# BirchKwok/lynsedb

Hardware: AMD Instinct MI355X
Metric: queries/sec, FLAT-IP 10000000x768 float32, batch=256, k=10 (higher is better)
Workload: dtype f32

## Files before the change

### lynsedb_amd/csrc/lynse_hip.hip

```cpp
#include <algorithm>
#include <atomic>
#include <chrono>
#include <cmath>
#include <cstdio>
#include <cstring>
#include <functional>
#include <condition_variable>
#include <memory>
#include <mutex>
#include <shared_mutex>
#include <string>
#include <thread>
#include <type_traits>
#include <vector>
#include <sched.h>

#include "kernels.h"
#include "scan_qs.h"
#include "scan_qh.h"
#include "ivf.h"
#include "pq.h"
#include "rabitq.h"
#include "range.h"
#include "additive.h"
// ... 913 lines not shown
    size_t seen = granted.load(std::memory_order_acquire);
    if (bytes <= seen) return LYNSE_OK;
    for (;;) {
        LY_TRY(set_max_lds(K, bytes));
        if (granted.compare_exchange_strong(seen, bytes, std::memory_order_acq_rel, std::memory_order_acquire)) return LYNSE_OK;
        bytes = std::max(bytes, seen);
    }
}
template <auto K, typename... Args>
static int launch_lds(dim3 grid, dim3 block, size_t lds, hipStream_t st, const Args&... a) {
    LY_TRY(ensure_lds<K>(lds));
    hipLaunchKernelGGL(K, grid, block, lds, st, a...);
    LY_HIP(hipGetLastError());
    return LYNSE_OK;
}

template <H16Cfg C>
static int launch_h16(dim3 grid, hipStream_t st, const ScanArgs& a) {
    return launch_lds<k_scan_h16<C.wq, C.wr, C.tq, C.tr, C.metric, C.nsv, C.nsq, C.nt_hint, C.tiled, C.rag, C.dbg, C.filt, C.i8q, C.emit, C.place, C.dense, C.prio, C.qcreg, C.fs>>(
        grid, h16_threads(C), h16_lds_bytes(C), st, a);
}
template <QsCfg C>
static int launch_qs(dim3 grid, hipStream_t st, const ScanArgs& a) {
    return launch_lds<k_scan_qs<C.nslab, C.rb, C.sl, C.ns, C.xpf, C.nbuf, C.dbg, C.ping, C.sts, C.met, C.smp, C.msk, C.f4>>(grid, QS_THREADS, qs_lds_bytes(C), st, a);
}
template <QhCfg C>
static int launch_qh(dim3 grid, hipStream_t st, const ScanArgs& a) {
    return launch_lds<k_scan_qh<C.nslab, C.met, C.ns, C.nbuf, C.qb, C.smp>>(grid, QH_THREADS, qh_lds_bytes(C), st, a);
}
template <class C, class T, class V, class... More>
constexpr C with(C c, T C::*member, V value, More... more) {
    c.*member = value;
    if constexpr (sizeof...(more) > 0) return with(c, more...);
    else return c;
}
template <class F>
static int with_metric(int metric, F&& f) {
    switch (metric) {
    case M_IP: return f(std::integral_constant<int, M_IP>{});
    case M_L2: return f(std::integral_constant<int, M_L2>{});
    default: return f(std::integral_constant<int, M_COS>{});
    }
}
template <H16Cfg BASE, int... VALUES>
static int dispatch_dbg(int dbg, dim3 grid, hipStream_t st, const ScanArgs& a) {
    int rc = LYNSE_OK;
    const bool known = (... || (dbg == VALUES ? (rc = launch_h16<with(BASE, &H16Cfg::dbg, VALUES)>(grid, st, a), true) : false));
// ... 327 lines not shown
    if (only768 || qs_variant() != 1) return false;
    if (!qs_widths_on()) return false;
    return ((nslab >= 2 && nslab <= 5) || nslab == 8) && ld == nslab * 128u;
}
static bool sts_env_on() { return env_on("LYNSE_HIP_STS", false); }
static bool qs_scan_ok(const ScanArgs& a, bool fs, bool filt, bool f4) {
    const int v = qs_variant();
    if (v < 1 || v > 3) return false;
    if (filt && (!qs_masked_on() || v == 2 || !a.mask || a.row_ids)) return false;
    if (f4) {
        return env_on("LYNSE_HIP_QS_F4", true) && v == 1 && !fs && !filt && a.emit_all == 0 && (a.nslab == 2 || a.nslab == 4 || a.nslab == 8) && a.ld16 == a.nslab * 128u &&
               a.qpad == 256 && a.nq <= 256 &&
               a.tile_stride == 0 && !a.mask && !a.row_ids && a.row1 > a.row0;
    }
    return !fs && a.emit_all == 0 && qs_width_ok(a.ld16, a.nslab, filt) && a.qpad == 256 && a.nq <= 256 && a.tile_stride == 0 &&
           (filt || (a.skip_stride == 0 && !a.mask)) && !a.row_ids && a.row1 > a.row0;
}
static uint32_t qs_grid(const ScanArgs& a, uint32_t num_cu) {
    const uint32_t rt = a.nslab == 8 ? 32u : qs_rows(qs_variant());
    const int e = env_int("LYNSE_HIP_SCAN_CUS", 0);
    const uint32_t cus = e > 0 ? std::min<uint32_t>((uint32_t)e, num_cu) : num_cu;
    return std::min<uint32_t>((a.row1 - a.row0 + rt - 1) / rt, cus);
}
static int launch_scan_qs(const ScanArgs& a, uint32_t grid, hipStream_t st) {
    if (a.dyn_thr)
        return launch_qs<with(QS_768, &QsCfg::ping, 0, &QsCfg::sts, 1)>(grid, st, a);
    if (a.mask) return launch_qs<with(QS_768, &QsCfg::msk, 1)>(grid, st, a);
    if (a.nslab >= 2 && a.nslab <= 5)
        return with_qs_slabs(a.nslab, [&](auto n) { return launch_qs<qs_64(decltype(n)::value)>(grid, st, a); });
    if (a.nslab == 8) return launch_qs<QS_1024>(grid, st, a);
    switch (qs_variant()) {
    case 2: return launch_qs<QsCfg{.nslab = 6, .rb = 1, .sl = 6, .ns = 6, .xpf = true, .nbuf = 8}>(grid, st, a);
    case 3: return launch_qs<with(QS_768, &QsCfg::ping, 0)>(grid, st, a);
    default: return launch_qs<QS_768>(grid, st, a);
    }
}

static bool qs_sample_ok(const ScanArgs& a, bool fs, bool filt, bool f4, uint32_t plan_tile) {
    const int v = qs_variant();
    if (!env_on("LYNSE_HIP_QS_SAMPLE", true) || (v != 1 && v != 3)) return false;
    return !fs && !filt && !f4 && a.emit_all == 2 && plan_tile == 256 && a.nslab != 8 && qs_width_ok(a.ld16, a.nslab) && a.qpad == 256 && a.nq <= 256 && a.tile_stride >= 256 &&
           a.skip_stride == 0 && !a.mask && !a.row_ids && a.row1 > a.row0;
}
static int launch_scan_qs_sample(const ScanArgs& a, uint32_t grid, hipStream_t st) {
    return with_qs_slabs(a.nslab, [&](auto n) { return launch_qs<with(qs_64(decltype(n)::value), &QsCfg::ping, 0, &QsCfg::smp, 1)>(grid, st, a); });
}

constexpr int QH_DEFAULT = 1;
static int qh_variant() { return env_int("LYNSE_HIP_QH", QH_DEFAULT); }
static bool qh_shape(uint32_t ld16, uint64_t nq) { return qh_variant() == 1 && nq > SCAN_BQ_SMALL && nq <= QCHUNK && (ld16 == 64u || ld16 == 128u); }
// ... 11 lines not shown
static int launch_scan_qh_any(const ScanArgs& a, int metric, uint32_t grid, hipStream_t st) {
    auto by_metric = [&](auto n) {
        return with_metric(metric, [&](auto m) { return launch_qh<qh_64(decltype(n)::value, decltype(m)::value, SMP)>(grid, st, a); });
    };
    return a.nslab == 1 ? by_metric(std::integral_constant<int, 1>{}) : by_metric(std::integral_constant<int, 2>{});
}
static int launch_scan_qh(const ScanArgs& a, int metric, uint32_t grid, hipStream_t st) { return launch_scan_qh_any<0>(a, metric, grid, st); }

static bool qh_sample_ok(const ScanArgs& a, bool filt, uint32_t qchunks, int level, uint32_t plan_tile) {
    if (!env_on("LYNSE_HIP_QH_SAMPLE", true) || qh_variant() != 1 || level != 0) return false;
    return !filt && a.emit_all == 2 && plan_tile == 256 && qchunks == 1 && a.qpad == 256 && a.nq <= 256 && a.tile_stride >= 256 && a.skip_stride == 0 && !a.mask && !a.row_ids &&
           !a.tiles && a.row1 > a.row0 && (a.nslab == 1 || a.nslab == 2) && a.ld16 == a.nslab * 64u;
}
static uint32_t qh_sample_grid(const ScanArgs& a, uint32_t sample_tiles, bool filt, uint32_t qchunks, int level, uint32_t plan_tile, uint32_t k, uint32_t cap, uint32_t num_cu) {
    if (!sample_tiles || !qh_sample_ok(a, filt, qchunks, level, plan_tile)) return 0;
    const uint32_t nt64 = sample_tiles * 4u, sgrid = std::min<uint32_t>(nt64, 2u * num_cu);
    const bool ok = (uint64_t)sgrid * 4u >= 8ull * k && sgrid * 4u <= cap && (nt64 + sgrid - 1) / sgrid <= 32u;
    return ok ? sgrid : 0u;
}
static int launch_scan_qh_sample(const ScanArgs& a, int metric, uint32_t grid, hipStream_t st) { return launch_scan_qh_any<1>(a, metric, grid, st); }

constexpr H16Cfg I8C_256 = with(F16_IP_256, &H16Cfg::rag, false, &H16Cfg::i8q, 2, &H16Cfg::emit, 0);
constexpr H16Cfg I8C_AG = with(I8C_256, &H16Cfg::wr, 2, &H16Cfg::tr, 4);
static int launch_scan_i8c(const ScanArgs& a, uint32_t grid, hipStream_t st, bool fs = false, bool filt = false, bool f4 = false, bool qs = false) {
    if (qs && f4) {
        if (a.nslab == 2) return launch_qs<with(qs_64(2), &QsCfg::f4, 1)>(grid, st, a);
        if (a.nslab == 8) return launch_qs<with(QS_1024, &QsCfg::f4, 1)>(grid, st, a);
        return launch_qs<with(qs_64(4), &QsCfg::f4, 1)>(grid, st, a);
    }
    if (qs) return launch_scan_qs(a, grid, st);
#ifdef LYNSE_EXPERIMENTS
    if (a.ld16 % 128 == 0 && a.emit_all == 0 && ((a.debug_flags >> 8) & 31)) {
        return dispatch_dbg<I8C_256, 3, 4, 8, 12, 7, 11, 1, 13, 14, 2, 16>((a.debug_flags >> 8) & 31, grid, st, a);
    }
#endif
    if (f4) {
        if (a.ld16 % 128 != 0 || filt || fs) return set_error(LYNSE_ERR_INTERNAL, "the FP4 Hamming scan runs unfiltered over whole slabs");
        if (a.emit_all == 1) return launch_h16<with(I8C_256, &H16Cfg::i8q, 3, &H16Cfg::emit, 1)>(grid, st, a);
        if (a.emit_all == 2) return launch_h16<with(I8C_256, &H16Cfg::i8q, 3, &H16Cfg::emit, 2)>(grid, st, a);
        if (a.dense) return launch_h16<with(I8C_256, &H16Cfg::i8q, 3, &H16Cfg::dense, true)>(grid, st, a);
        return launch_h16<with(I8C_256, &H16Cfg::i8q, 3)>(grid, st, a);
    }
    if (filt) {
        if (a.ld16 % 128 != 0 || a.row_ids) return set_error(LYNSE_ERR_INTERNAL, "the masked int8 scan needs whole 128-column slabs and a row bitmask");
        if (a.emit_all == 1) return launch_h16<with(I8C_256, &H16Cfg::filt, true, &H16Cfg::emit, 1)>(grid, st, a);
        if (a.emit_all != 0 || !a.dense) return set_error(LYNSE_ERR_INTERNAL, "the masked int8 scan runs emit-all and DENSE threshold stages");
        return launch_h16<with(I8C_256, &H16Cfg::filt, true, &H16Cfg::dense, true)>(grid, st, a);
    }
    if (ag_env() && a.ld16 % 128 == 0 && a.emit_all == 0 && !fs) {
        if (a.dense) return launch_h16<with(I8C_AG, &H16Cfg::dense, true)>(grid, st, a);
        return launch_h16<I8C_AG>(grid, st, a);
    }
    if (a.ld16 % 128 == 0) {
// ... 242 lines not shown
#else
    constexpr int w16env = -1;
#endif
    const bool filt = mask != nullptr || row_ids != nullptr;
    const int waves16 = l2n ? 0 : i8c ? 3 : (w16env >= 0 ? w16env : ((metric == M_IP && !filt) ? 3 : 0));
    const bool can_threshold_only = h16 && !binary && !filt && !no_lane_max_env() && k <= 128;
    Stage assign_stage{0u, (uint32_t)h->n};
    assign_stage.sample_tiles = (uint32_t)((h->n + 255) / 256);
    assign_stage.sample_stride = 256;
    const std::vector<Stage> plan = tl_assign ? std::vector<Stage>{assign_stage}
                                    : (sts || tl_coarse_dump) ? std::vector<Stage>{Stage{0u, (uint32_t)h->n}}
                                        : make_plan(h, k, (level == 0 && (!plan_tile || no_sample)) ? 1 : level, plan_tile, can_threshold_only,
                                                    (h16 && !i8c && !binary && k >= 64) ? 4u : 0u);
    const Stage sample = (!plan.empty() && plan[0].sample_tiles) ? plan[0] : Stage{0, 0};
    *sampled_plan = sample.sample_tiles != 0;
    const uint32_t sample_keys_per_tile = (small || mid64 || mid128 || waves16 != 0) ? 16u : 8u;
    const bool sample_threshold_only = h16 && !binary && !filt && sample.sample_tiles && !no_lane_max_env() && sample_keys_per_tile &&
                                       (k <= sample_keys_per_tile || (uint64_t)sample.sample_tiles * sample_keys_per_tile >= 8ull * k);
    const int fs_env = fused_sample_env();
    const bool fs = fs_env != 0 && !debug_flags_env() && i8c && !aug && !cosq && !l2n && !bin_mfma && !mid64 && !mid128 && h->ld8 % 128 == 0 && sample_threshold_only && plan.size() >= 2 && k <= 32 &&
                    sample.sample_tiles == (uint32_t)h->num_cu && (plan[1].r1 - plan[1].r0 + 255) / 256 >= (uint32_t)h->num_cu &&
                    (uint64_t)k * 50000ull > (uint64_t)sample.sample_tiles * plan_tile &&
                    dense_env_now() != 0;
    bool plan_used_segments = false, plan_used_qs = false, plan_qs_sample = false, plan_used_qh = false;
    const int fused_tail_env = env_int("LYNSE_HIP_FUSED_TAIL", 1);
    const bool fused_tail = fused_tail_env != 0 && !plan.empty();
    SelectArgs sa_last{};
    for (size_t si = 0; si < plan.size(); ++si) {
        const Stage s = plan[si];
        const bool emit_all = si == 0 && !sts;
        if (fs && si == 0) continue;
        const bool fs_stage = fs && si == 1;
        uint32_t qs_sample_keys = 0;
        hipEvent_t e0 = nullptr, e1 = nullptr;
        if (tl_prof) {
            LY_TRY(get_event(h, (*ev_used)++, &e0));
            LY_TRY(get_event(h, (*ev_used)++, &e1));
            LY_HIP(hipEventRecord(e0, st));
        }
        uint32_t st_nseg = 0, st_seg = 0;
        int a_emit_all_last = -1;
        if (binary && !bin_mfma) {
            BinArgs b{};
            b.P = h->packed; b.W = h->words; b.row0 = s.r0; b.row1 = s.r1; b.QW = w.QW; b.nq = nq;
            b.thr = w.thr; b.cand = w.cand; b.count = w.count; b.cap = w.cap; b.emit_all = emit_all ? 1 : 0;
            b.mask = mask;
            static const int rows_minq = env_int("LYNSE_HIP_BIN_ROWS_MINQ", 1);
// ... 84 lines not shown
                    a.dyn_warm = h->n >= 4000000ull ? 4u : 2u;
                }
                if (s.sample_tiles && !sts && qs_sample_ok(a, fs_stage, filt, bin_mfma, plan_tile)) {
                    const uint32_t nt64 = s.sample_tiles * 4u;
                    const uint32_t sgrid = std::min<uint32_t>(nt64, (uint32_t)h->num_cu);
                    if ((uint64_t)sgrid * 4u >= 8ull * k && sgrid * 4u <= w.cap && (nt64 + sgrid - 1) / sgrid <= 32u) {
                        a.ntiles = nt64;
                        LY_TRY(launch_scan_qs_sample(a, sgrid, st));
                        qs_sample_keys = sgrid * 4u;
                        plan_qs_sample = true;
                    }
                }
                if (!qs_sample_keys) {
                const bool qs = sts || (!ag && qs_scan_ok(a, fs_stage, filt, bin_mfma));
                uint32_t launch_grid = qs ? qs_grid(a, (uint32_t)h->num_cu) : grid;
                if (sts) {
                    const uint32_t nt = (a.row1 - a.row0 + 63) / 64;
                    uint32_t pitch = (nt + launch_grid - 1) / launch_grid;
                    auto gcd = [](uint32_t x, uint32_t y) { while (y) { const uint32_t t = x % y; x = y; y = t; } return x; };
                    while (gcd(pitch, k) != 1) ++pitch;
                    a.dyn_pitch = pitch;
                    launch_grid = (nt + pitch - 1) / pitch;
                }
                if (qs) { seg_geometry(launch_grid, 2, &a.nseg, &a.seg); plan_used_qs = true; }
                else
                if (!a.emit_all) seg_geometry(grid, (a.dense ? 8 : 4) / (ag ? 2 : 1), &a.nseg, &a.seg);
                if (fs_stage) {
                    a.fs_stride = sample.sample_stride; a.fs_rows = (uint32_t)h->n; a.gsync = w.gsync; a.Qf = Qf; a.marg2 = w.marg2;
                    a.thr_out = w.thr; a.k = k; a.ip_form = ip_form; a.metric = metric;
                    if (env_str("LYNSE_HIP_FS_STAMPS")) a.debug_flags |= 128;
                }
                LY_TRY(launch_scan_i8c(a, launch_grid, st, fs_stage, filt, bin_mfma, qs));
                }
            } else if (h16) {
                a.candB = w.candB; a.segcnt = w.segcnt;
                if (small) {
                    const uint32_t grid = std::min<uint32_t>(a.ntiles, (uint32_t)h->num_cu * 2);
                    if (!a.emit_all) seg_geometry(grid, 4, &a.nseg, &a.seg);
                    LY_TRY((launch_scan_h16<F16_SMALL>(a, metric, grid, st)));
                } else if (const uint32_t sgrid = qh_sample_grid(a, s.sample_tiles, filt, qchunks, level, plan_tile, k, w.cap, (uint32_t)h->num_cu)) {
                    a.ntiles = s.sample_tiles * 4u;
                    LY_TRY(launch_scan_qh_sample(a, metric, sgrid, st));
                    qs_sample_keys = sgrid * 4u;
                    plan_used_qh = true;
                } else if (qh_scan_ok(a, filt, qchunks, level)) {
                    uint32_t segs = 0;
                    const uint32_t grid = qh_grid(a, (uint32_t)h->num_cu, &segs);
                    seg_geometry(grid, segs, &a.nseg, &a.seg);
                    plan_used_qh = true;
                    LY_TRY(launch_scan_qh(a, metric, grid, st));
                } else {
                    const uint32_t grid = std::min<uint32_t>(a.ntiles, (uint32_t)h->num_cu);
                    const uint64_t seen_before = s.sample_tiles ? 0 : (sample.sample_tiles ? std::max<uint64_t>((uint64_t)sample.sample_tiles * plan_tile, s.r0) : s.r0);
                    a.dense = (!a.emit_all && waves16 == 0 && metric != M_IP && !filt && seen_before && (dense_env() >= 0 ? dense_env() != 0 : true)) ? 1 : 0;
                    if (!a.emit_all) seg_geometry(grid, a.dense ? 4 : ((waves16 == 3 || waves16 == 2) ? 4 : 2), &a.nseg, &a.seg);
// ... 64 lines not shown
        sa.emit_all_n = emit_all ? (s.sample_tiles ? (int)(s.sample_tiles * plan_tile) : (int)(s.r1 - s.r0)) : -1;
        if (!binary && emit_all && sample_threshold_only) {
            sa.threshold_only = 1;
            sa.drop_sentinels = 1;
            sa.emit_all_n = qs_sample_keys ? (int)qs_sample_keys : (int)(s.sample_tiles * sample_keys_per_tile);
        }
        sa.Qf = Qf; sa.V = score_rows(h); sa.ld = score_ld(h); sa.D = h->dim;
        sa.candB = w.candB; sa.segcnt = w.segcnt; sa.seg = st_seg; sa.nseg = st_nseg;
        sa.abort_word = fs_stage ? w.gsync + 2 : nullptr;
        if (sel_stamps_on())
            sa.stamps = reinterpret_cast<unsigned long long*>(w.gsync + 64) + (size_t)si * 256 * 8;
        if (fs_stage && env_str("LYNSE_HIP_DEBUG_FS")) return LYNSE_OK;
        if (fused_tail && si + 1 == plan.size()) { sa_last = sa; continue; }
        sa.lds_bytes = sel_lds_bytes(w.cap, nq);
        hipLaunchKernelGGL(k_select<SEL_NT>, dim3(nq), dim3(SEL_NT), sa.lds_bytes, st, sa);
        LY_HIP(hipGetLastError());
    }
    if (tl_prof && (!binary || bin_mfma)) {
        const uint64_t tiling = plan_used_qs ? 0x81u : plan_used_qh ? 0x82u : (small || mid64) ? 0x14u : ((mid128 || waves16 == 3 || waves16 == 2) ? 0x24u : 0x42u);
        std::lock_guard<std::mutex> plk(h->prof_mu);
        h->prof.last_plan = (sample.sample_tiles ? 1u : 0u) | ((sample.sample_tiles && sample_threshold_only) ? 2u : 0u) | (i8c ? 4u : 0u) |
                            (plan_used_segments ? 8u : 0u) | (small ? 16u : 0u) | (fs ? 128u : 0u) | ((uint64_t)(plan.size() & 0xff) << 8) | (tiling << 16) |
                            (sts ? (1ull << 24) : 0ull) | (plan_qs_sample ? (1ull << 25) : 0ull) |
                            (sq7 ? (1ull << 26) : 0ull);
    }
    FinalArgs fa{};
    fa.cand = w.cand; fa.count = w.count; fa.k = k; fa.out_k = out_k; fa.cap = w.cap; fa.metric = key_metric; fa.ip_form = ip_form;
    fa.ham_dim = bin_mfma ? h->dim : 0u;
    fa.neg_metric1 = (aug || cosq) ? metric + 1 : 0;
    fa.exact = binary ? 1 : 0; fa.Qf = Qf; fa.V = score_rows(h); fa.ld = score_ld(h); fa.D = h->dim;
    fa.row_stride = h->row_stride; fa.row_offset = h->row_offset;
    fa.nan_rows = (!binary && !mask && !row_ids && h->n <= 0xffffffffull) ? (uint32_t)h->n : 0u;
    fa.out_rows = r_dst ? r_dst : w.out_rows; fa.out_dists = d_dst ? d_dst : w.out_dists; fa.out_counts = w.out_counts;
    fa.out_counts2 = c2_dst;
    fa.pool_total = tl_prof ? w.pool_total : nullptr;
    fa.overflow = w.overflow; fa.any_overflow = any_ovf;
    if (hdr_direct) { fa.h_hdr = w.h_hdr; fa.hdr_q = w.qcap; }
    if (fused_tail) {
        TailArgs ta{sa_last, fa};
        ta.s.hand_exact = env_int("LYNSE_HIP_HAND_EXACT", 1);
        ta.s.lds_bytes = ta.f.lds_bytes = sel_lds_bytes(w.cap, nq);
        hipLaunchKernelGGL(k_select_final<SEL_NT>, dim3(nq), dim3(SEL_NT), ta.s.lds_bytes, st, ta);
        LY_HIP(hipGetLastError());
        (void)asc;
        return LYNSE_OK;
    }
    if (i8c && !bin_mfma) {
// ... 1406 lines not shown
```

### lynsedb_amd/csrc/scan_qs.h

```cpp
#pragma once

namespace lynse {

typedef int qs_i32x4 __attribute__((ext_vector_type(4)));
typedef int qs_i32x16 __attribute__((ext_vector_type(16)));

constexpr int QS_STS_LDS = 8 * 256 + 8 * 256;

struct QsCfg {
    int nslab, rb, sl, ns;
    bool xpf;
    int nbuf;
    int dbg = 0, ping = 0, sts = 0, met = 0, smp = 0, msk = 0, f4 = 0;
};
constexpr int QS_THREADS = 512;
constexpr size_t qs_lds_bytes(QsCfg c) {
    const size_t norm_slot = c.met == 1 ? (c.rb * 32 == 64 ? 256 : 1024) : 0;
    return (size_t)c.ns * c.sl * (c.rb * 32) * 128 + (c.sts ? QS_STS_LDS : 0) + (size_t)(c.ns + 1) * norm_slot;
}

template <int NSLAB, int RB, int SL, int NS, bool XPF, int NBUF, int DBG = 0, int PING = 0, int STS = 0, int MET = 0, int SMP = 0, int MSK = 0, int F4 = 0>
__global__ void __launch_bounds__(512, 2) k_scan_qs(ScanArgs a) {
    static_assert(NSLAB % SL == 0, "a tile is a whole number of steps");
    constexpr int TS = NSLAB / SL;
    constexpr int RT = RB * 32;
    constexpr int SB = SL * RT * 128;
    constexpr int PP = SB / 1024;
    static_assert(PP % 8 == 0, "the pieces of a stage split evenly over the 8 waves");
    constexpr int PPW = PP / 8;
    constexpr int NM = SL * 4 * RB;
    static_assert(NM % NBUF == 0 && NBUF >= 2 && NBUF <= NM, "fragment ring");
    static_assert(NS >= (XPF ? 4 : 3), "ring depth");
    constexpr int NRM = MET == 1 ? (RT == 64 ? 256 : 1024) : 0;
    constexpr int NRM_SLOTS = NS + 1;
    constexpr int NRM_OFF = NS * SB + (STS ? QS_STS_LDS : 0);
    static_assert(MET == 0 || (STS == 0 && TS == 1 && RT <= 256), "L2: whole-K stages; one dword / dwordx4 LDS-DMA brings a tile's norms");
    static_assert(NRM_OFF + NRM_SLOTS * NRM <= 160 * 1024, "LDS");
    static_assert((size_t)(NRM_OFF + NRM_SLOTS * NRM) <= qs_lds_bytes(QsCfg{NSLAB, RB, SL, NS, XPF, NBUF, DBG, PING, STS, MET, SMP, MSK, F4}),
                  "the LDS the body addresses ends inside what the launch asks for");
    static_assert(PING == 0 || TS == 1, "ping-pong: one step per tile");
    static_assert(STS == 0 || (!XPF && TS == 1), "self-tightening thresholds: whole-K stages, no cross-barrier prefetch");
    static_assert(SMP == 0 || (STS == 0 && MET == 0 && RT == 64 && TS == 1), "sample stage: 64-row tiles of the IP / cosine form");
    static_assert(MSK == 0 || (STS == 0 && MET == 0 && SMP == 0), "masked threshold stages: the IP / cosine form");
    static_assert(F4 == 0 || (STS == 0 && MET == 0 && SMP == 0 && MSK == 0 && DBG == 0), "FP4 Hamming: plain threshold stages");
    constexpr int WAITN = (XPF ? NS - 3 : NS - 2) * PPW;
    static_assert(WAITN <= 63, "vmcnt");

    extern __shared__ __attribute__((aligned(16))) char smem[];
    const int tid = threadIdx.x, lane = tid & 63;
    const int wave = __builtin_amdgcn_readfirstlane(tid >> 6);
    const int l32 = lane & 31, hi = lane >> 5;
    const uint32_t ntiles = SMP != 0 ? a.ntiles : (a.row1 - a.row0 + RT - 1) / RT;
    auto tile_row0 = [&](uint32_t t) -> uint32_t {
        if constexpr (SMP != 0) return a.row0 + (t >> 2) * a.tile_stride + (t & 3u) * (uint32_t)RT;
        else return a.row0 + t * RT;
    };
    const uint32_t pitch = STS != 0 ? a.dyn_pitch : 0u;
    uint32_t my_tiles;
    if constexpr (STS != 0) {
        if ((uint64_t)blockIdx.x * pitch >= ntiles) return;
        my_tiles = ntiles - blockIdx.x * pitch < pitch ? ntiles - blockIdx.x * pitch : pitch;
    } else {
        if (blockIdx.x >= ntiles) return;
        my_tiles = (ntiles - blockIdx.x + gridDim.x - 1) / gridDim.x;
    }
    uint32_t warm = 0;
    if constexpr (STS != 0) warm = a.dyn_warm * 4u <= my_tiles ? a.dyn_warm : my_tiles / 4u;
    const uint32_t n_ord = my_tiles + warm;
    const uint32_t G = n_ord * TS;
    [[maybe_unused]] const unsigned long long t_kernel0 = (a.debug_flags & 64) ? __builtin_amdgcn_s_memtime() : 0ull;
    auto tile_of = [&](uint32_t ord) -> uint32_t {
        const uint32_t i = ord < my_tiles ? ord : ord - my_tiles;
        if constexpr (STS != 0) return blockIdx.x * pitch + i;
        else return blockIdx.x + i * gridDim.x;
    };

    const int swz = (l32 >> 1) & 7;
    qs_i32x4 bq[NSLAB * 4];
    {
        const char* qimg = reinterpret_cast<const char*>(a.Q16) + (size_t)(wave * 32 + l32) * 128;
#pragma unroll
        for (int s = 0; s < NSLAB; ++s)
#pragma unroll
            for (int kk = 0; kk < 4; ++kk)
                bq[s * 4 + kk] = *reinterpret_cast<const qs_i32x4*>(qimg + (size_t)s * a.qpad * 128 + (((kk * 2 + hi) ^ swz) * 16));
    }
    const uint32_t qn = wave * 32 + l32;
    const bool q_ok = qn < a.nq;
    const bool wave_live = (uint32_t)wave * 32u < a.nq;
    const float s_q = q_ok ? a.qinv[qn] : 0.0f, b_q = q_ok ? a.qn2[qn] : 0.0f;
    [[maybe_unused]] const float thr_q = (q_ok && STS == 0 && SMP == 0) ? a.thr[qn] : 0.0f;
    asm volatile("" ::: "memory");
    [[maybe_unused]] unsigned long long smp_t[4] = {0ull, 0ull, 0ull, 0ull}, smp_rt = 0ull;
    [[maybe_unused]] const bool smp_stamps = SMP != 0 && (a.debug_flags & 64) != 0;
    if constexpr (SMP != 0) { if (smp_stamps) smp_rt = __builtin_amdgcn_s_memrealtime(); }

    uint32_t v_off[PPW];
    const char* v_base = nullptr;
    uint32_t is_ord = 0, is_sub = 0, is_stage = 0, is_count = 0;
    auto enter_tile = [&]() {
        const uint32_t rbase = tile_row0(tile_of(is_ord));
        const uint32_t span = a.row1 - 1 - rbase;
        v_base = reinterpret_cast<const char*>(a.V16) + (size_t)rbase * a.ld16;
#pragma unroll
        for (int j = 0; j < PPW; ++j) {
            const int p = wave * PPW + j;
            uint32_t r = (p % (RB * 4)) * 8 + (lane >> 3);
            const uint32_t col = (uint32_t)(p / (RB * 4)) * 128u + (((lane & 7) ^ ((r >> 1) & 7)) * 16);
            r = r < span ? r : span;
            v_off[j] = r * a.ld16 + col;
        }
    };
    auto issue_piece = [&](int j) {
        if (DBG & 8) return;
// ... 22 lines not shown
    enter_tile();
#pragma unroll
    for (int s0 = 0; s0 < NS - 1; ++s0) {
#pragma unroll
        for (int j = 0; j < PPW; ++j) issue_piece(j);
        issue_norms();
        advance();
    }
    if constexpr (SMP != 0) { if (smp_stamps) smp_t[0] = __builtin_amdgcn_s_memtime(); }

    int T = 0x7fffffff;
    [[maybe_unused]] float l2_thr = 0.0f, l2_pre = LY_INF, l2_2s = 0.0f;
    if constexpr (MET == 1) {
        l2_thr = q_ok ? thr_q : -LY_INF;
        l2_2s = 2.0f * s_q;
        const float vmax2 = a.vmax2;
        float pre = (b_q - l2_thr) - 2e-6f * (b_q + fabsf(l2_thr) + vmax2);
        if (!(vmax2 > 0.0f) || !(fabsf(pre) < 3.0e38f)) pre = -LY_INF;
        l2_pre = q_ok ? pre : LY_INF;
#ifdef LYNSE_EXPERIMENTS
        if (a.debug_flags & 2) l2_pre = LY_INF;
#endif
    }
    if constexpr (STS == 0 && MET == 0 && SMP == 0) {
        const float th = thr_q;
        int lo = -(1 << 29), hi_ = 1 << 29;
#pragma unroll 1
        for (int it = 0; it < 31; ++it) {
            const int mid = lo + ((hi_ - lo) >> 1);
            const bool ge = (b_q + s_q * (float)mid) >= th;
            hi_ = ge ? mid : hi_;
            lo = ge ? lo : mid + 1;
        }
        T = q_ok ? lo : 0x7fffffff;
#ifdef LYNSE_EXPERIMENTS
        if (a.debug_flags & 2) T = 0x7fffffff;
#endif
    }
    [[maybe_unused]] int tau_c = -2147483647 - 1, dyn_m = 0, pub_last = -2147483647 - 1;
    [[maybe_unused]] int* const land_thr = reinterpret_cast<int*>(smem + NS * SB) + wave * 64 + lane;
    [[maybe_unused]] int* const land_slot = reinterpret_cast<int*>(smem + NS * SB + 8 * 256) + wave * 64 + lane;
    [[maybe_unused]] const int* thr_src = nullptr;
    [[maybe_unused]] const int* slot_src = nullptr;
    [[maybe_unused]] const uint32_t hq = blockIdx.x + (uint32_t)wave * gridDim.x;
    [[maybe_unused]] const bool helper = STS != 0 && hq < a.nq;
    [[maybe_unused]] uint32_t sts_step = 0;
// ... 5 lines not shown
#endif
        return tau_c < -(1 << 30) ? -(1 << 30) - (1 << 29) : tau_c - dyn_m;
    };
    if constexpr (STS != 0) {
        thr_src = a.dyn_thr + (q_ok ? qn : 0u);
        slot_src = a.dyn_slot + (size_t)(helper ? hq : 0u) * 32 + l32;
        dyn_m = q_ok ? a.dyn_marg[qn] : 0;
        tau_c = __hip_atomic_load(thr_src, __ATOMIC_RELAXED, __HIP_MEMORY_SCOPE_SYSTEM);
        *land_thr = tau_c;
        *land_slot = -2147483647 - 1;
        T = sts_T();
    }
    if constexpr (MET == 1) {
        if (wave == 0) asm volatile("s_waitcnt vmcnt(%0) lgkmcnt(0)" ::"n"((NS - 1) * PPW + (NS - 1)) : "memory");
        else asm volatile("s_waitcnt vmcnt(%0) lgkmcnt(0)" ::"n"((NS - 1) * PPW) : "memory");
    } else if constexpr ((DBG & 8) != 0 || STS != 0) {
        asm volatile("s_waitcnt vmcnt(0) lgkmcnt(0)" ::: "memory");
    } else {
        asm volatile("s_waitcnt vmcnt(%0) lgkmcnt(0)" ::"n"((NS - 1) * PPW) : "memory");
    }
    if constexpr (SMP != 0) { if (smp_stamps) smp_t[1] = __builtin_amdgcn_s_memtime(); }

    const uint32_t lds0 = (uint32_t)(uintptr_t)(__attribute__((address_space(3))) char*)smem;
    const uint32_t a_lane = lds0 + (uint32_t)l32 * 128u + (uint32_t)((hi ^ swz) * 16);
    qs_i32x4 af[NBUF];
    auto read_frag = [&](qs_i32x4& dst, const uint32_t (&ad)[4], auto idxc) {
        constexpr int idx = decltype(idxc)::value;
        constexpr int sl = idx / (4 * RB), kk = (idx / RB) % 4, rb = idx % RB;
#ifdef LYNSE_QS_AF_AGPR
        asm volatile("ds_read_b128 %0, %1 offset:%2" : "=a"(dst) : "v"(ad[kk]), "n"(sl * (RT * 128) + rb * (32 * 128)));
#else
        asm volatile("ds_read_b128 %0, %1 offset:%2" : "=v"(dst) : "v"(ad[kk]), "n"(sl * (RT * 128) + rb * (32 * 128)));
#endif
    };
    using acc_t = std::conditional_t<F4 != 0, f32x16, qs_i32x16>;
    acc_t acc[RB];
#pragma unroll
    for (int i = 0; i < RB; ++i)
#pragma unroll
        for (int r = 0; r < 16; ++r) acc[i][r] = 0;
    [[maybe_unused]] int f4_unit = 0x7f7f7f7f;
    if constexpr (F4 != 0) asm volatile("" : "+v"(f4_unit));

    uint32_t cnt = 0;
    uint32_t c_ord = 0;
    uint32_t c_stage = 0;
    uint32_t ad_cur[4], ad_nxt[4];
#pragma unroll
    for (int kk = 0; kk < 4; ++kk) ad_nxt[kk] = a_lane ^ (uint32_t)(kk * 32);
    if constexpr (XPF) {
        asm volatile("s_waitcnt vmcnt(%0)" ::"n"((NS - 2) * PPW) : "memory");
        __builtin_amdgcn_s_barrier();
        if (!(DBG & 2)) ly_static_for<NBUF - 1>([&](auto ic) { read_frag(af[decltype(ic)::value], ad_nxt, ic); });
    }
    constexpr bool TIMING = (DBG & 32) != 0;
    [[maybe_unused]] unsigned long long t_wait = 0, t_bar = 0, t_loop = 0, t_epi = 0, tp = TIMING ? __builtin_amdgcn_s_memtime() : 0ull;
    [[maybe_unused]] auto stamp = [&](unsigned long long& bucket) {
        if constexpr (TIMING) { const unsigned long long t = __builtin_amdgcn_s_memtime(); bucket += t - tp; tp = t; }
    };
    auto mfma_step = [&](auto sc, auto dma_in) {
        constexpr int s = decltype(sc)::value;
        constexpr bool DMA_IN = decltype(dma_in)::value;
        if constexpr (!XPF) {
            if (!(DBG & 2)) ly_static_for<NBUF - 1>([&](auto ic) { read_frag(af[decltype(ic)::value], ad_cur, ic); });
        }
        __builtin_amdgcn_sched_barrier(0);
        ly_static_for<NM>([&](auto ic) {
            constexpr int idx = decltype(ic)::value;
            constexpr int nxt = idx + NBUF - 1;
            if (!(DBG & 2)) {
                if constexpr (nxt < NM) read_frag(af[nxt % NBUF], ad_cur, std::integral_constant<int, nxt>{});
                else if constexpr (XPF) read_frag(af[nxt % NBUF], ad_nxt, std::integral_constant<int, nxt - NM>{});
                constexpr int outstanding = (nxt < NM || XPF) ? NBUF : NM - idx;
#ifdef LYNSE_QS_AF_AGPR
                asm volatile("s_waitcnt lgkmcnt(%1)" : "+a"(af[idx % NBUF]) : "n"(outstanding - 1));
#else
                asm volatile("s_waitcnt lgkmcnt(%1)" : "+v"(af[idx % NBUF]) : "n"(outstanding - 1));
#endif
            }
            __builtin_amdgcn_sched_barrier(0);
            constexpr int sl = idx / (4 * RB), kk = (idx / RB) % 4, rb = idx % RB;
            constexpr int ks = (s * SL + sl) * 4 + kk;
            if constexpr ((DBG & 1) != 0) {
                asm volatile("" ::"v"(af[idx % NBUF]), "v"(bq[ks]));
            } else if constexpr ((DBG & 128) != 0) {
                qs_i32x4 c0 = __builtin_shufflevector(acc[rb], acc[rb], 0, 1, 2, 3), c1 = __builtin_shufflevector(acc[rb], acc[rb], 4, 5, 6, 7);
                c0 = __builtin_amdgcn_mfma_i32_16x16x64_i8(af[idx % NBUF], bq[ks], c0, 0, 0, 0);
                c1 = __builtin_amdgcn_mfma_i32_16x16x64_i8(af[idx % NBUF], bq[ks], c1, 0, 0, 0);
                acc[rb][0] = c0[0]; acc[rb][1] = c0[1]; acc[rb][2] = c0[2]; acc[rb][3] = c0[3];
                acc[rb][4] = c1[0]; acc[rb][5] = c1[1]; acc[rb][6] = c1[2]; acc[rb][7] = c1[3];
            } else if constexpr (F4 != 0) {
                if constexpr (ks == 0) {
                    const f32x16 z = {0, 0, 0, 0, 0, 0, 0, 0, 0, 0, 0, 0, 0, 0, 0, 0};
                    acc[rb] = ly_mfma_fp4(af[idx % NBUF], bq[ks], z, f4_unit);
                } else {
                    acc[rb] = ly_mfma_fp4(af[idx % NBUF], bq[ks], acc[rb], f4_unit);
                }
            } else if constexpr (ks == 0) {
                const qs_i32x16 z = {0, 0, 0, 0, 0, 0, 0, 0, 0, 0, 0, 0, 0, 0, 0, 0};
                acc[rb] = __builtin_amdgcn_mfma_i32_32x32x32_i8(af[idx % NBUF], bq[ks], z, 0, 0, 0);
            } else {
                acc[rb] = __builtin_amdgcn_mfma_i32_32x32x32_i8(af[idx % NBUF], bq[ks], acc[rb], 0, 0, 0);
            }
            if constexpr (DMA_IN) {
                ly_static_for<PPW>([&](auto jc) {
                    constexpr int j = decltype(jc)::value;
                    if constexpr (idx == (NM / PPW) * j + 1) issue_piece(j);
                });
            }
            __builtin_amdgcn_sched_barrier(0);
        });
    };
    [[maybe_unused]] uint32_t sts_extra = 0;
    auto wait_and_barrier = [&]() {
        if constexpr (MET == 1) {
            if (wave == 0) asm volatile("s_waitcnt vmcnt(%0)" ::"n"(WAITN + (XPF ? NS - 3 : NS - 2)) : "memory");
            else asm volatile("s_waitcnt vmcnt(%0)" ::"n"(WAITN) : "memory");
        } else if constexpr (STS != 0) {
            if (sts_extra == 0) asm volatile("s_waitcnt vmcnt(%0)" ::"n"(WAITN) : "memory");
            else if (sts_extra == 1) asm volatile("s_waitcnt vmcnt(%0)" ::"n"(WAITN + 1) : "memory");
            else asm volatile("s_waitcnt vmcnt(%0)" ::"n"(WAITN + 2) : "memory");
        } else {
            asm volatile("s_waitcnt vmcnt(%0)" ::"n"(WAITN) : "memory");
        }
        stamp(t_wait);
        __builtin_amdgcn_s_barrier();
        stamp(t_bar);
        if constexpr (STS != 0) {
            asm volatile("ds_read_b32 %0, %1" : "=v"(peek_thr) : "v"((uint32_t)(uintptr_t)(__attribute__((address_space(3))) const int*)land_thr) : "memory");
            if (helper) asm volatile("ds_read_b32 %0, %1" : "=v"(peek_slot) : "v"((uint32_t)(uintptr_t)(__attribute__((address_space(3))) const int*)land_slot) : "memory");
        }
        c_stage = c_stage + 1 == NS ? 0 : c_stage + 1;
#pragma unroll
        for (int kk = 0; kk < 4; ++kk) {
            ad_cur[kk] = ad_nxt[kk];
            ad_nxt[kk] = (a_lane ^ (uint32_t)(kk * 32)) + c_stage * SB;
        }
    };
    [[maybe_unused]] auto sts_refresh = [&]() {
        const uint32_t s = sts_step++;
        sts_extra = 0;
#ifdef LYNSE_EXPERIMENTS
        if ((a.debug_flags & 256) && s >= 16u) return;
#endif
        if (s < 16u || (s & 3u) == 0u) {
            sts_extra = helper ? 2u : 1u;
            constexpr int AUX = STS == 1 ? 17 : (STS == 2 ? 16 : 0);
            __builtin_amdgcn_global_load_lds((const __attribute__((address_space(1))) void*)thr_src,
                                             (__attribute__((address_space(3))) void*)(reinterpret_cast<int*>(smem + NS * SB) + wave * 64), 4, 0, AUX);
            if (helper)
                __builtin_amdgcn_global_load_lds((const __attribute__((address_space(1))) void*)slot_src,
                                                 (__attribute__((address_space(3))) void*)(reinterpret_cast<int*>(smem + NS * SB + 8 * 256) + wave * 64), 4, 0, AUX);
        }
    };
    [[maybe_unused]] auto sts_pickup = [&]() {
        asm volatile("s_waitcnt lgkmcnt(0)" : "+v"(peek_thr), "+v"(peek_slot)::"memory");
        const int seen = peek_thr;
        tau_c = seen > tau_c ? seen : tau_c;
        T = sts_T();
        if (helper && (sts_step < 20u || (sts_step & 3u) == 3u)) {
            int m = peek_slot;
#pragma unroll
            for (int o = 16; o > 0; o >>= 1) { const int t2 = __shfl_xor(m, o, 64); m = t2 < m ? t2 : m; }
            if (lane == 0 && m > pub_last) { atomicMax(a.dyn_thr + hq, m); pub_last = m; }
        }
    };
    [[maybe_unused]] int smp1 = -2147483647 - 1, smp2 = -2147483647 - 1;
    auto epilogue = [&](uint32_t e_tile, bool emit, [[maybe_unused]] uint32_t e_ord_) {
        if constexpr (SMP != 0) {
            const uint32_t rbase = tile_row0(e_tile);
            const int pos0 = (int)((e_ord_ & 31u) << 5);
            const bool whole = rbase + RT <= a.row1;
#pragma unroll
            for (int i = 0; i < RB; ++i)
#pragma unroll
                for (int r = 0; r < 16; ++r) {
                    int t = (acc[i][r] & ~1023) | (pos0 | (i * 16 + r));
                    if (!whole) {
                        const uint32_t m = rbase + i * 32 + (r & 3) + 8 * (r >> 2) + 4 * hi;
                        t = m < a.row1 ? t : -2147483647 - 1;
                    }
                    const int lo3 = smp1 < t ? smp1 : t, hi3 = smp1 < t ? t : smp1;
                    smp2 = smp2 > lo3 ? smp2 : lo3;
                    smp1 = hi3;
                }
        } else if constexpr ((DBG & 16) != 0) {
#pragma unroll
            for (int i = 0; i < RB; ++i)
#pragma unroll
                for (int r = 0; r < 16; ++r) asm volatile("" ::"v"(acc[i][r]));
        } else if constexpr (MET == 1) {
            const uint32_t nbase = lds0 + NRM_OFF + (e_ord_ % NRM_SLOTS) * NRM + (uint32_t)hi * 16u;
// ... 168 lines not shown
                    stamp(t_loop);
                    pend = true;
                }
            }
        }
    }
    if constexpr (SMP != 0) {
        if (smp_stamps) smp_t[3] = __builtin_amdgcn_s_memtime();
        if (q_ok) {
#pragma unroll
            for (int t = 0; t < 2; ++t) {
                const uint32_t slot = (blockIdx.x * 2 + hi) * 2 + t;
                const int pk = t == 0 ? smp1 : smp2;
                uint64_t key = KEY_SENTINEL;
                if (pk != -2147483647 - 1) {
                    const uint32_t pos = (uint32_t)pk & 1023u, r = pos & 15u;
                    const uint32_t m = tile_row0(tile_of(pos >> 5)) + ((pos >> 4) & 1u) * 32u + (r & 3u) + 8u * (r >> 2) + 4u * (uint32_t)hi;
                    key = make_key(b_q + s_q * (float)(pk & ~1023), m, false);
                }
                if (slot < a.cap) a.cand[(size_t)qn * a.cap + slot] = key;
            }
        }
    }
    if (a.seg && q_ok) a.segcnt[(size_t)qn * a.nseg + (blockIdx.x * 2 + hi)] = (uint8_t)cnt;
    if constexpr (TIMING) {
        if (a.dbg && lane == 0 && blockIdx.x < 64) {
            unsigned long long* o = a.dbg + 2 * 256 + ((size_t)blockIdx.x * 8 + wave) * 4;
            o[0] = t_wait; o[1] = t_bar; o[2] = t_loop; o[3] = t_epi;
        }
    }
    if constexpr (SMP != 0) {
        if (smp_stamps && a.dbg && tid == 0) {
            asm volatile("s_waitcnt vmcnt(0)" ::: "memory");
            unsigned long long* o = a.dbg + (size_t)blockIdx.x * 8;
            o[0] = t_kernel0; o[1] = smp_t[0]; o[2] = smp_t[1]; o[3] = smp_t[2]; o[4] = smp_t[3]; o[5] = __builtin_amdgcn_s_memtime(); o[6] = smp_rt;
        }
    } else
    if ((a.debug_flags & 64) && a.dbg && tid == 0) {
        a.dbg[blockIdx.x * 2] = t_kernel0;
        a.dbg[blockIdx.x * 2 + 1] = __builtin_amdgcn_s_memtime();
    }
    asm volatile("s_waitcnt vmcnt(0)" ::: "memory");
}

}
```

Baseline: 141,800.

## Add 16x16x64 int8 MFMA variant of the QS threshold scan

Adds an M16 template variant of the quantized-scan kernel. It computes dot products with 16x16x64 int8 MFMA instructions instead of the 32x32 form, using a new query-fragment layout, per-16-query thresholds, and a new epilogue that writes four segments per workgroup. It is enabled by default for plain threshold stages, unless the LYNSE_HIP_QS_M16 environment variable is set to 0. The intent is a more efficient MFMA shape and finer-grained emit, at the cost of more accumulator registers, more segments, and a more complex epilogue.

New measurement: 150,700 (median of 6 runs). 1.06x the previous value.

```diff
diff --git a/lynsedb_amd/csrc/lynse_hip.hip b/lynsedb_amd/csrc/lynse_hip.hip
--- a/lynsedb_amd/csrc/lynse_hip.hip
+++ b/lynsedb_amd/csrc/lynse_hip.hip
@@ -959,7 +959,7 @@
 }
 template <QsCfg C>
 static int launch_qs(dim3 grid, hipStream_t st, const ScanArgs& a) {
-    return launch_lds<k_scan_qs<C.nslab, C.rb, C.sl, C.ns, C.xpf, C.nbuf, C.dbg, C.ping, C.sts, C.met, C.smp, C.msk, C.f4>>(grid, QS_THREADS, qs_lds_bytes(C), st, a);
+    return launch_lds<k_scan_qs<C.nslab, C.rb, C.sl, C.ns, C.xpf, C.nbuf, C.dbg, C.ping, C.sts, C.met, C.smp, C.msk, C.f4, C.m16>>(grid, QS_THREADS, qs_lds_bytes(C), st, a);
 }
 template <QhCfg C>
 static int launch_qh(dim3 grid, hipStream_t st, const ScanArgs& a) {
@@ -1333,10 +1333,19 @@
     const uint32_t cus = e > 0 ? std::min<uint32_t>((uint32_t)e, num_cu) : num_cu;
     return std::min<uint32_t>((a.row1 - a.row0 + rt - 1) / rt, cus);
 }
-static int launch_scan_qs(const ScanArgs& a, uint32_t grid, hipStream_t st) {
+static int qs_m16_env() { return env_int("LYNSE_HIP_QS_M16", -1); }
+static bool qs_m16_stage(const ScanArgs& a, bool sts, bool filt, bool f4) {
+    if (qs_m16_env() == 0 || qs_variant() != 1) return false;
+    return !sts && !filt && !f4 && !a.mask && !a.dyn_thr && a.nslab >= 2 && a.nslab <= 6;
+}
+static int launch_scan_qs(const ScanArgs& a, uint32_t grid, hipStream_t st, bool m16 = false) {
     if (a.dyn_thr)
         return launch_qs<with(QS_768, &QsCfg::ping, 0, &QsCfg::sts, 1)>(grid, st, a);
     if (a.mask) return launch_qs<with(QS_768, &QsCfg::msk, 1)>(grid, st, a);
+    if (m16) {
+        if (a.nseg != 0 && a.nseg != grid * 4u) return set_error(LYNSE_ERR_INTERNAL, "the 16x16x64 scan needs four segments per workgroup and query");
+        return with_qs_slabs(a.nslab, [&](auto n) { return launch_qs<with(qs_64(decltype(n)::value), &QsCfg::m16, 1)>(grid, st, a); });
+    }
     if (a.nslab >= 2 && a.nslab <= 5)
         return with_qs_slabs(a.nslab, [&](auto n) { return launch_qs<qs_64(decltype(n)::value)>(grid, st, a); });
     if (a.nslab == 8) return launch_qs<QS_1024>(grid, st, a);
@@ -1394,13 +1403,13 @@
 
 constexpr H16Cfg I8C_256 = with(F16_IP_256, &H16Cfg::rag, false, &H16Cfg::i8q, 2, &H16Cfg::emit, 0);
 constexpr H16Cfg I8C_AG = with(I8C_256, &H16Cfg::wr, 2, &H16Cfg::tr, 4);
-static int launch_scan_i8c(const ScanArgs& a, uint32_t grid, hipStream_t st, bool fs = false, bool filt = false, bool f4 = false, bool qs = false) {
+static int launch_scan_i8c(const ScanArgs& a, uint32_t grid, hipStream_t st, bool fs = false, bool filt = false, bool f4 = false, bool qs = false, bool m16 = false) {
     if (qs && f4) {
         if (a.nslab == 2) return launch_qs<with(qs_64(2), &QsCfg::f4, 1)>(grid, st, a);
         if (a.nslab == 8) return launch_qs<with(QS_1024, &QsCfg::f4, 1)>(grid, st, a);
         return launch_qs<with(qs_64(4), &QsCfg::f4, 1)>(grid, st, a);
     }
-    if (qs) return launch_scan_qs(a, grid, st);
+    if (qs) return launch_scan_qs(a, grid, st, m16);
 #ifdef LYNSE_EXPERIMENTS
     if (a.ld16 % 128 == 0 && a.emit_all == 0 && ((a.debug_flags >> 8) & 31)) {
         return dispatch_dbg<I8C_256, 3, 4, 8, 12, 7, 11, 1, 13, 14, 2, 16>((a.debug_flags >> 8) & 31, grid, st, a);
@@ -1689,7 +1698,7 @@
                     sample.sample_tiles == (uint32_t)h->num_cu && (plan[1].r1 - plan[1].r0 + 255) / 256 >= (uint32_t)h->num_cu &&
                     (uint64_t)k * 50000ull > (uint64_t)sample.sample_tiles * plan_tile &&
                     dense_env_now() != 0;
-    bool plan_used_segments = false, plan_used_qs = false, plan_qs_sample = false, plan_used_qh = false;
+    bool plan_used_segments = false, plan_used_qs = false, plan_qs_sample = false, plan_used_qh = false, plan_qs_m16 = false;
     const int fused_tail_env = env_int("LYNSE_HIP_FUSED_TAIL", 1);
     const bool fused_tail = fused_tail_env != 0 && !plan.empty();
     SelectArgs sa_last{};
@@ -1820,7 +1829,8 @@
                     a.dyn_pitch = pitch;
                     launch_grid = (nt + pitch - 1) / pitch;
                 }
-                if (qs) { seg_geometry(launch_grid, 2, &a.nseg, &a.seg); plan_used_qs = true; }
+                const bool m16 = qs && qs_m16_stage(a, sts, filt, bin_mfma);
+                if (qs) { seg_geometry(launch_grid, m16 ? 4 : 2, &a.nseg, &a.seg); plan_used_qs = true; plan_qs_m16 = plan_qs_m16 || m16; }
                 else
                 if (!a.emit_all) seg_geometry(grid, (a.dense ? 8 : 4) / (ag ? 2 : 1), &a.nseg, &a.seg);
                 if (fs_stage) {
@@ -1828,7 +1838,7 @@
                     a.thr_out = w.thr; a.k = k; a.ip_form = ip_form; a.metric = metric;
                     if (env_str("LYNSE_HIP_FS_STAMPS")) a.debug_flags |= 128;
                 }
-                LY_TRY(launch_scan_i8c(a, launch_grid, st, fs_stage, filt, bin_mfma, qs));
+                LY_TRY(launch_scan_i8c(a, launch_grid, st, fs_stage, filt, bin_mfma, qs, m16));
                 }
             } else if (h16) {
                 a.candB = w.candB; a.segcnt = w.segcnt;
@@ -1939,7 +1949,8 @@
         h->prof.last_plan = (sample.sample_tiles ? 1u : 0u) | ((sample.sample_tiles && sample_threshold_only) ? 2u : 0u) | (i8c ? 4u : 0u) |
                             (plan_used_segments ? 8u : 0u) | (small ? 16u : 0u) | (fs ? 128u : 0u) | ((uint64_t)(plan.size() & 0xff) << 8) | (tiling << 16) |
                             (sts ? (1ull << 24) : 0ull) | (plan_qs_sample ? (1ull << 25) : 0ull) |
-                            (sq7 ? (1ull << 26) : 0ull);
+                            (sq7 ? (1ull << 26) : 0ull) |
+                            (plan_qs_m16 ? (1ull << 27) : 0ull);
     }
     FinalArgs fa{};
     fa.cand = w.cand; fa.count = w.count; fa.k = k; fa.out_k = out_k; fa.cap = w.cap; fa.metric = key_metric; fa.ip_form = ip_form;
diff --git a/lynsedb_amd/csrc/scan_qs.h b/lynsedb_amd/csrc/scan_qs.h
--- a/lynsedb_amd/csrc/scan_qs.h
+++ b/lynsedb_amd/csrc/scan_qs.h
@@ -11,7 +11,7 @@
     int nslab, rb, sl, ns;
     bool xpf;
     int nbuf;
-    int dbg = 0, ping = 0, sts = 0, met = 0, smp = 0, msk = 0, f4 = 0;
+    int dbg = 0, ping = 0, sts = 0, met = 0, smp = 0, msk = 0, f4 = 0, m16 = 0;
 };
 constexpr int QS_THREADS = 512;
 constexpr size_t qs_lds_bytes(QsCfg c) {
@@ -19,7 +19,7 @@
     return (size_t)c.ns * c.sl * (c.rb * 32) * 128 + (c.sts ? QS_STS_LDS : 0) + (size_t)(c.ns + 1) * norm_slot;
 }
 
-template <int NSLAB, int RB, int SL, int NS, bool XPF, int NBUF, int DBG = 0, int PING = 0, int STS = 0, int MET = 0, int SMP = 0, int MSK = 0, int F4 = 0>
+template <int NSLAB, int RB, int SL, int NS, bool XPF, int NBUF, int DBG = 0, int PING = 0, int STS = 0, int MET = 0, int SMP = 0, int MSK = 0, int F4 = 0, int M16 = 0>
 __global__ void __launch_bounds__(512, 2) k_scan_qs(ScanArgs a) {
     static_assert(NSLAB % SL == 0, "a tile is a whole number of steps");
     constexpr int TS = NSLAB / SL;
@@ -36,13 +36,17 @@
     constexpr int NRM_OFF = NS * SB + (STS ? QS_STS_LDS : 0);
     static_assert(MET == 0 || (STS == 0 && TS == 1 && RT <= 256), "L2: whole-K stages; one dword / dwordx4 LDS-DMA brings a tile's norms");
     static_assert(NRM_OFF + NRM_SLOTS * NRM <= 160 * 1024, "LDS");
-    static_assert((size_t)(NRM_OFF + NRM_SLOTS * NRM) <= qs_lds_bytes(QsCfg{NSLAB, RB, SL, NS, XPF, NBUF, DBG, PING, STS, MET, SMP, MSK, F4}),
+    static_assert((size_t)(NRM_OFF + NRM_SLOTS * NRM) <= qs_lds_bytes(QsCfg{NSLAB, RB, SL, NS, XPF, NBUF, DBG, PING, STS, MET, SMP, MSK, F4, M16}),
                   "the LDS the body addresses ends inside what the launch asks for");
     static_assert(PING == 0 || TS == 1, "ping-pong: one step per tile");
     static_assert(STS == 0 || (!XPF && TS == 1), "self-tightening thresholds: whole-K stages, no cross-barrier prefetch");
     static_assert(SMP == 0 || (STS == 0 && MET == 0 && RT == 64 && TS == 1), "sample stage: 64-row tiles of the IP / cosine form");
     static_assert(MSK == 0 || (STS == 0 && MET == 0 && SMP == 0), "masked threshold stages: the IP / cosine form");
     static_assert(F4 == 0 || (STS == 0 && MET == 0 && SMP == 0 && MSK == 0 && DBG == 0), "FP4 Hamming: plain threshold stages");
+    static_assert(M16 == 0 || (STS == 0 && MET == 0 && F4 == 0 && SMP == 0 && (DBG & 32) == 0), "16x16x64 form: threshold stages of the IP / cosine form");
+    constexpr int R16 = RT / 16;
+    constexpr int NKK = M16 != 0 ? 2 : 4;
+    constexpr int KX = M16 != 0 ? 64 : 32;
     constexpr int WAITN = (XPF ? NS - 3 : NS - 2) * PPW;
     static_assert(WAITN <= 63, "vmcnt");
 
@@ -76,8 +80,18 @@
     };
 
     const int swz = (l32 >> 1) & 7;
+    [[maybe_unused]] const int c16 = lane & 15, g4 = lane >> 4, swz16 = (c16 >> 1) & 7;
     qs_i32x4 bq[NSLAB * 4];
-    {
+    if constexpr (M16 != 0) {
+#pragma unroll
+        for (int s = 0; s < NSLAB; ++s)
+#pragma unroll
+            for (int k64 = 0; k64 < 2; ++k64)
+#pragma unroll
+                for (int qb = 0; qb < 2; ++qb)
+                    bq[s * 4 + k64 * 2 + qb] = *reinterpret_cast<const qs_i32x4*>(reinterpret_cast<const char*>(a.Q16) + (size_t)(wave * 32 + qb * 16 + c16) * 128 +
+                                                                                  (size_t)s * a.qpad * 128 + (((k64 * 4 + g4) ^ swz16) * 16));
+    } else {
         const char* qimg = reinterpret_cast<const char*>(a.Q16) + (size_t)(wave * 32 + l32) * 128;
 #pragma unroll
         for (int s = 0; s < NSLAB; ++s)
@@ -90,6 +104,19 @@
     const bool wave_live = (uint32_t)wave * 32u < a.nq;
     const float s_q = q_ok ? a.qinv[qn] : 0.0f, b_q = q_ok ? a.qn2[qn] : 0.0f;
     [[maybe_unused]] const float thr_q = (q_ok && STS == 0 && SMP == 0) ? a.thr[qn] : 0.0f;
+    [[maybe_unused]] uint32_t qn16[2] = {0u, 0u};
+    [[maybe_unused]] bool q_ok16[2] = {false, false};
+    [[maybe_unused]] float s_q16[2] = {0.0f, 0.0f}, b_q16[2] = {0.0f, 0.0f}, thr_q16[2] = {0.0f, 0.0f};
+    if constexpr (M16 != 0) {
+#pragma unroll
+        for (int qb = 0; qb < 2; ++qb) {
+            qn16[qb] = (uint32_t)(wave * 32 + qb * 16 + c16);
+            q_ok16[qb] = qn16[qb] < a.nq;
+            s_q16[qb] = q_ok16[qb] ? a.qinv[qn16[qb]] : 0.0f;
+            b_q16[qb] = q_ok16[qb] ? a.qn2[qn16[qb]] : 0.0f;
+            thr_q16[qb] = q_ok16[qb] ? a.thr[qn16[qb]] : 0.0f;
+        }
+    }
     asm volatile("" ::: "memory");
     [[maybe_unused]] unsigned long long smp_t[4] = {0ull, 0ull, 0ull, 0ull}, smp_rt = 0ull;
     [[maybe_unused]] const bool smp_stamps = SMP != 0 && (a.debug_flags & 64) != 0;
@@ -158,6 +185,27 @@
         if (a.debug_flags & 2) l2_pre = LY_INF;
 #endif
     }
+    [[maybe_unused]] int T16[2] = {0x7fffffff, 0x7fffffff};
+    if constexpr (M16 != 0) {
+        int lo[2] = {-(1 << 29), -(1 << 29)}, hi_[2] = {1 << 29, 1 << 29};
+#pragma unroll 1
+        for (int it = 0; it < 31; ++it) {
+#pragma unroll
+            for (int qb = 0; qb < 2; ++qb) {
+                const int mid = lo[qb] + ((hi_[qb] - lo[qb]) >> 1);
+                const bool ge = (b_q16[qb] + s_q16[qb] * (float)mid) >= thr_q16[qb];
+                hi_[qb] = ge ? mid : hi_[qb];
+                lo[qb] = ge ? lo[qb] : mid + 1;
+            }
+        }
+#pragma unroll
+        for (int qb = 0; qb < 2; ++qb) {
+            T16[qb] = q_ok16[qb] ? lo[qb] : 0x7fffffff;
+#ifdef LYNSE_EXPERIMENTS
+            if (a.debug_flags & 2) T16[qb] = 0x7fffffff;
+#endif
+        }
+    } else
     if constexpr (STS == 0 && MET == 0 && SMP == 0) {
         const float th = thr_q;
         int lo = -(1 << 29), hi_ = 1 << 29;
@@ -209,10 +257,19 @@
     if constexpr (SMP != 0) { if (smp_stamps) smp_t[1] = __builtin_amdgcn_s_memtime(); }
 
     const uint32_t lds0 = (uint32_t)(uintptr_t)(__attribute__((address_space(3))) char*)smem;
-    const uint32_t a_lane = lds0 + (uint32_t)l32 * 128u + (uint32_t)((hi ^ swz) * 16);
+    const uint32_t a_lane = M16 != 0 ? lds0 + (uint32_t)c16 * 128u + (uint32_t)((g4 ^ swz16) * 16) : lds0 + (uint32_t)l32 * 128u + (uint32_t)((hi ^ swz) * 16);
     qs_i32x4 af[NBUF];
+    if constexpr ((DBG & 2) != 0) {
+#pragma unroll
+        for (int i = 0; i < NBUF; ++i) asm volatile("" : "=v"(af[i]) : "0"(bq[i]));
+    }
     auto read_frag = [&](qs_i32x4& dst, const uint32_t (&ad)[4], auto idxc) {
         constexpr int idx = decltype(idxc)::value;
+        if constexpr (M16 != 0) {
+            constexpr int sl16 = idx / (2 * R16), k64 = (idx / R16) % 2, rb16 = idx % R16;
+            asm volatile("ds_read_b128 %0, %1 offset:%2" : "=v"(dst) : "v"(ad[k64]), "n"(sl16 * (RT * 128) + rb16 * (16 * 128)));
+            return;
+        }
         constexpr int sl = idx / (4 * RB), kk = (idx / RB) % 4, rb = idx % RB;
 #ifdef LYNSE_QS_AF_AGPR
         asm volatile("ds_read_b128 %0, %1 offset:%2" : "=a"(dst) : "v"(ad[kk]), "n"(sl * (RT * 128) + rb * (32 * 128)));
@@ -229,12 +286,18 @@
     [[maybe_unused]] int f4_unit = 0x7f7f7f7f;
     if constexpr (F4 != 0) asm volatile("" : "+v"(f4_unit));
 
+    [[maybe_unused]] qs_i32x4 acc16[R16][2];
+#pragma unroll
+    for (int i = 0; i < R16; ++i)
+#pragma unroll
+        for (int qb = 0; qb < 2; ++qb) acc16[i][qb] = qs_i32x4{0, 0, 0, 0};
+    [[maybe_unused]] uint32_t cnt16[2] = {0u, 0u};
     uint32_t cnt = 0;
     uint32_t c_ord = 0;
     uint32_t c_stage = 0;
     uint32_t ad_cur[4], ad_nxt[4];
 #pragma unroll
-    for (int kk = 0; kk < 4; ++kk) ad_nxt[kk] = a_lane ^ (uint32_t)(kk * 32);
+    for (int kk = 0; kk < 4; ++kk) ad_nxt[kk] = a_lane ^ (uint32_t)((kk % NKK) * KX);
     if constexpr (XPF) {
         asm volatile("s_waitcnt vmcnt(%0)" ::"n"((NS - 2) * PPW) : "memory");
         __builtin_amdgcn_s_barrier();
@@ -270,12 +333,18 @@
             constexpr int ks = (s * SL + sl) * 4 + kk;
             if constexpr ((DBG & 1) != 0) {
                 asm volatile("" ::"v"(af[idx % NBUF]), "v"(bq[ks]));
-            } else if constexpr ((DBG & 128) != 0) {
-                qs_i32x4 c0 = __builtin_shufflevector(acc[rb], acc[rb], 0, 1, 2, 3), c1 = __builtin_shufflevector(acc[rb], acc[rb], 4, 5, 6, 7);
-                c0 = __builtin_amdgcn_mfma_i32_16x16x64_i8(af[idx % NBUF], bq[ks], c0, 0, 0, 0);
-                c1 = __builtin_amdgcn_mfma_i32_16x16x64_i8(af[idx % NBUF], bq[ks], c1, 0, 0, 0);
-                acc[rb][0] = c0[0]; acc[rb][1] = c0[1]; acc[rb][2] = c0[2]; acc[rb][3] = c0[3];
-                acc[rb][4] = c1[0]; acc[rb][5] = c1[1]; acc[rb][6] = c1[2]; acc[rb][7] = c1[3];
+            } else if constexpr (M16 != 0) {
+                constexpr int k64 = (idx / R16) % 2, rb16 = idx % R16;
+                constexpr int kb = (s * SL + idx / (2 * R16)) * 4 + k64 * 2;
+                ly_static_for<2>([&](auto qbc) {
+                    constexpr int qb = decltype(qbc)::value;
+                    if constexpr (kb == 0) {
+                        const qs_i32x4 z = {0, 0, 0, 0};
+                        acc16[rb16][qb] = __builtin_amdgcn_mfma_i32_16x16x64_i8(af[idx % NBUF], bq[kb + qb], z, 0, 0, 0);
+                    } else {
+                        acc16[rb16][qb] = __builtin_amdgcn_mfma_i32_16x16x64_i8(af[idx % NBUF], bq[kb + qb], acc16[rb16][qb], 0, 0, 0);
+                    }
+                });
             } else if constexpr (F4 != 0) {
                 if constexpr (ks == 0) {
                     const f32x16 z = {0, 0, 0, 0, 0, 0, 0, 0, 0, 0, 0, 0, 0, 0, 0, 0};
@@ -321,7 +390,7 @@
 #pragma unroll
         for (int kk = 0; kk < 4; ++kk) {
             ad_cur[kk] = ad_nxt[kk];
-            ad_nxt[kk] = (a_lane ^ (uint32_t)(kk * 32)) + c_stage * SB;
+            ad_nxt[kk] = (a_lane ^ (uint32_t)((kk % NKK) * KX)) + c_stage * SB;
         }
     };
     [[maybe_unused]] auto sts_refresh = [&]() {
@@ -354,7 +423,61 @@
     };
     [[maybe_unused]] int smp1 = -2147483647 - 1, smp2 = -2147483647 - 1;
     auto epilogue = [&](uint32_t e_tile, bool emit, [[maybe_unused]] uint32_t e_ord_) {
-        if constexpr (SMP != 0) {
+        if constexpr (M16 != 0 && (DBG & 16) != 0) {
+#pragma unroll
+            for (int i = 0; i < R16; ++i)
+#pragma unroll
+                for (int qb = 0; qb < 2; ++qb)
+#pragma unroll
+                    for (int r = 0; r < 4; ++r) asm volatile("" ::"v"(acc16[i][qb][r]));
+        } else if constexpr (M16 != 0) {
+            int gm[R16][2];
+#pragma unroll
+            for (int i = 0; i < R16; ++i)
+#pragma unroll
+                for (int qb = 0; qb < 2; ++qb) {
+                    const qs_i32x4 v = acc16[i][qb];
+                    const int m01 = v[0] > v[1] ? v[0] : v[1];
+                    const int m012 = m01 > v[2] ? m01 : v[2];
+                    gm[i][qb] = m012 > v[3] ? m012 : v[3];
+                }
+            int mx[2] = {gm[0][0], gm[0][1]};
+#pragma unroll
+            for (int i = 1; i < R16; ++i)
+#pragma unroll
+                for (int qb = 0; qb < 2; ++qb) mx[qb] = mx[qb] > gm[i][qb] ? mx[qb] : gm[i][qb];
+            if (__builtin_expect(__ballot(mx[0] >= T16[0] || mx[1] >= T16[1]) != 0ull, 0)) {
+                const uint32_t rbase = a.row0 + e_tile * RT;
+                if constexpr (MSK != 0) {
+                    if (a.skip_stride && rbase % a.skip_stride < 256u && rbase / a.skip_stride < a.skip_tiles) return;
+                }
+#pragma unroll
+                for (int i = 0; i < R16; ++i) {
+#pragma unroll
+                    for (int qb = 0; qb < 2; ++qb) {
+                        if (__builtin_expect(__ballot(gm[i][qb] >= T16[qb]) == 0ull, 1)) continue;
+                        uint64_t* segdst = a.candB + ((size_t)qn16[qb] * a.nseg + (blockIdx.x * 4 + g4)) * a.seg;
+#pragma unroll
+                        for (int e = 0; e < 4; ++e) {
+                            const int v = acc16[i][qb][e];
+                            if (v >= T16[qb]) {
+                                const uint32_t m = rbase + i * 16 + 4 * g4 + e;
+                                if (m < a.row1 && (MSK == 0 || ((a.mask[m >> 5] >> (m & 31)) & 1u))) {
+                                    const uint64_t key = make_key(b_q16[qb] + s_q16[qb] * (float)v, m, false);
+                                    if (cnt16[qb] < a.seg) {
+                                        segdst[cnt16[qb]] = key;
+                                        ++cnt16[qb];
+                                    } else {
+                                        const uint32_t slot = atomicAdd(&a.count[qn16[qb]], 1u);
+                                        if (slot < a.cap) a.cand[(size_t)qn16[qb] * a.cap + slot] = key;
+                                    }
+                                }
+                            }
+                        }
+                    }
+                }
+            }
+        } else if constexpr (SMP != 0) {
             const uint32_t rbase = tile_row0(e_tile);
             const int pos0 = (int)((e_ord_ & 31u) << 5);
             const bool whole = rbase + RT <= a.row1;
@@ -569,6 +692,11 @@
             }
         }
     }
+    if constexpr (M16 != 0) {
+#pragma unroll
+        for (int qb = 0; qb < 2; ++qb)
+            if (a.seg && q_ok16[qb]) a.segcnt[(size_t)qn16[qb] * a.nseg + (blockIdx.x * 4 + g4)] = (uint8_t)cnt16[qb];
+    } else
     if (a.seg && q_ok) a.segcnt[(size_t)qn * a.nseg + (blockIdx.x * 2 + hi)] = (uint8_t)cnt;
     if constexpr (TIMING) {
         if (a.dbg && lane == 0 && blockIdx.x < 64) {
```
